# k-xlsx/huff-encoding

Measured on AMD Instinct MI355X. Metric: encode+decode GB/s on 1 GiB bytes at 1/2/4/8 MI355X; % HBM roofline, higher is better.
Workload: dtype u8; 1 GPU; 1 GiB uniform bytes (BASELINE configs[1]), encode+decode, bit-exact; bytes_per_gpu=1073741824, global_bytes=1073741824, compressed_bytes_per_gpu=1073741824, parallelism=shard1

## Files before the change

huff-encoding_amd/csrc/device/indexless.hip:

```cpp
#include <algorithm>

#include "segwalk.hpp"

namespace huff::dev {

namespace {

constexpr int kThreads = 256;

struct Seg {
    const uint8_t* comp;
    uint64_t comp_bytes;
    uint64_t B;
    uint64_t S;
    uint64_t nseg;
    const uint32_t* lut;
    uint32_t K;
    unsigned long long* wtot;
};

__device__ __forceinline__ void load_prim(uint32_t* plut, const Seg& g) {
    for (uint32_t i = threadIdx.x; i < (1u << g.K); i += blockDim.x) plut[i] = g.lut[i];
    __syncthreads();
}
// ... 180 lines not shown
template <class Step>
__device__ __forceinline__ void fix_list_body(const Seg& g, const PackedRecs& R, uint64_t* __restrict__ x,
                                              unsigned int* __restrict__ flags, const uint32_t* __restrict__ list,
                                              uint32_t* __restrict__ chain, const Step& step) {
    const uint64_t firsts = (g.nseg - 1) / kThreads;
    const uint64_t n = firsts + __builtin_nontemporal_load(flags + kFixRounds);
    for (uint64_t j = static_cast<uint64_t>(blockIdx.x) * blockDim.x + threadIdx.x; j < n;
         j += static_cast<uint64_t>(gridDim.x) * blockDim.x) {
        const uint64_t i = j < firsts ? (j + 1) * kThreads : list[j - firsts];
        fix_one(g, R, x, flags, 0, i, step, chain, flags + kFixRounds + 1);
    }
}
__global__ __launch_bounds__(kThreads) void k_fix_list(Seg g, PackedRecs R, uint64_t* __restrict__ x,
                                                       unsigned int* __restrict__ flags,
                                                       const uint32_t* __restrict__ list, uint32_t* __restrict__ chain,
                                                       FixTabs f) {
    extern __shared__ uint32_t plut[];
    if (f.wt) {
        fix_list_body(g, R, x, flags, list, chain, load_len_step(f, plut));
    } else {
        load_prim(plut, g);
        fix_list_body(g, R, x, flags, list, chain, LutStep{Lut{plut, g.lut, g.K}});
    }
}

constexpr int kChainThreads = 1024;
template <class Step>
__device__ __forceinline__ void fix_chain_body(const Seg& g, const PackedRecs& R, uint64_t* __restrict__ x,
                                               unsigned int* __restrict__ flags, uint32_t* __restrict__ chain,
                                               const Step& step);
__global__ __launch_bounds__(kChainThreads) void k_fix_chain(Seg g, PackedRecs R, uint64_t* __restrict__ x,
                                                             unsigned int* __restrict__ flags,
                                                             uint32_t* __restrict__ chain, FixTabs f) {
    if (__builtin_nontemporal_load(flags + kFixRounds + 1) == 0) return;
    extern __shared__ uint32_t plut[];
    if (f.wt) {
        fix_chain_body(g, R, x, flags, chain, load_len_step(f, plut));
    } else {
        load_prim(plut, g);
        fix_chain_body(g, R, x, flags, chain, LutStep{Lut{plut, g.lut, g.K}});
    }
}
template <class Step>
__device__ __forceinline__ void fix_chain_body(const Seg& g, const PackedRecs& R, uint64_t* __restrict__ x,
                                               unsigned int* __restrict__ flags, uint32_t* __restrict__ chain,
                                               const Step& step) {
    __shared__ uint32_t n_sh;
    uint32_t cur = 0;
    for (;;) {
        unsigned int* cnt = flags + kFixRounds + 1 + cur;
        unsigned int* ncnt = flags + kFixRounds + 2 - cur;
        if (threadIdx.x == 0) n_sh = atomicAdd(cnt, 0u);
        __syncthreads();
        const uint32_t n = n_sh;
        if (n == 0) break;
        const uint32_t* list = chain + static_cast<uint64_t>(cur) * g.nseg;
        uint32_t* nl = chain + static_cast<uint64_t>(cur ^ 1u) * g.nseg;
        for (uint32_t j = threadIdx.x; j < n; j += blockDim.x) fix_one(g, R, x, flags, 0, list[j], step, nl, ncnt);
        __syncthreads();
        if (threadIdx.x == 0) {
            atomicExch(cnt, 0u);
            atomicAdd(flags + kFixRounds + 3, n);
        }
        cur ^= 1u;
    }
}

__global__ void k_settle(Seg g, uint64_t* __restrict__ s, uint64_t* __restrict__ x, uint64_t* __restrict__ c,
                         uint32_t* __restrict__ tm, const unsigned int* __restrict__ flags) {
    if (__builtin_nontemporal_load(flags + kFixRounds - 1) == 0) return;
    extern __shared__ uint32_t plut[];
    load_prim(plut, g);
    if (threadIdx.x != 0) return;
    const BitSrc src{reinterpret_cast<const uint32_t*>(g.comp), g.comp, g.comp_bytes};
    const Lut lut{plut, g.lut, g.K};
    for (uint64_t i = 1; i < g.nseg; ++i) {
        const uint64_t ns = x[i - 1];
        if (ns == s[i]) continue;
        const uint64_t end = (i + 1 == g.nseg) ? g.B : ((i + 1) * g.S < g.B ? (i + 1) * g.S : g.B);
        BitReader rd;
        rd.seek(src, ns);
        uint64_t cnt = 0;
        while (rd.pos < end) {
            if (!step(rd, src, lut, g.B)) break;
            ++cnt;
        }
        s[i] = ns;
        x[i] = rd.pos;
        if (g.wtot) g.wtot[i / kThreads] += cnt - c[i];
        c[i] = cnt;
        tm[i] = kNoMerge;
    }
}

__global__ __launch_bounds__(kThreads) void k_emit(Seg g, const uint64_t* __restrict__ s,
                                                   const uint64_t* __restrict__ c, const uint64_t* __restrict__ off,
                                                   uint8_t* __restrict__ out) {
    extern __shared__ uint32_t plut[];
    load_prim(plut, g);
    const uint64_t i = static_cast<uint64_t>(blockIdx.x) * blockDim.x + threadIdx.x;
    if (i >= g.nseg) return;
    const uint64_t cnt = c[i];
    if (cnt == 0) return;
    const BitSrc src{reinterpret_cast<const uint32_t*>(g.comp), g.comp, g.comp_bytes};
    const Lut lut{plut, g.lut, g.K};
    BitReader rd;
    rd.seek(src, s[i]);
    uint8_t* o = out + off[i];
    for (uint64_t j = 0; j < cnt; ++j) {
        const uint32_t e = rd.peek(src, lut);
        rd.advance(src, (e >> 8) & 0xFFu);
        o[j] = static_cast<uint8_t>(e);
    }
}

Seg make_seg(const IndexlessArgs& a) {
    return Seg{a.comp, a.comp_bytes, a.valid_bits, a.seg_bits, a.nseg, a.lut, a.lut_bits, a.wtot};
}


constexpr uint32_t kSampStride = (kSampMax + 1) & ~1u;
constexpr uint32_t kSampNone = 0xFFFFu;
struct SampWords {
    uint32_t d[kSampStride / 2];
};
typedef uint32_t u32x4_a4 __attribute__((ext_vector_type(4), aligned(4)));
__device__ __forceinline__ SampWords samp_load(const uint16_t* samp, uint64_t i) {
    SampWords w;
    const uint32_t* p = reinterpret_cast<const uint32_t*>(samp + i * kSampStride);
    constexpr uint32_t kD = kSampStride / 2;
    uint32_t k = 0;
#pragma unroll
    for (; k + 4 <= kD; k += 4) {
        const u32x4_a4 v = *reinterpret_cast<const u32x4_a4*>(p + k);
        w.d[k] = v.x;
        w.d[k + 1] = v.y;
        w.d[k + 2] = v.z;
        w.d[k + 3] = v.w;
    }
#pragma unroll
    for (; k < kD; ++k) w.d[k] = p[k];
    return w;
}
__device__ __forceinline__ void samp_store(uint16_t* samp, uint64_t i, const SampWords& w) {
    uint32_t* p = reinterpret_cast<uint32_t*>(samp + i * kSampStride);
    constexpr uint32_t kD = kSampStride / 2;
    uint32_t k = 0;
#pragma unroll
    for (; k + 4 <= kD; k += 4)
        *reinterpret_cast<u32x4_a4*>(p + k) = u32x4_a4{w.d[k], w.d[k + 1], w.d[k + 2], w.d[k + 3]};
#pragma unroll
    for (; k < kD; ++k) p[k] = w.d[k];
}
__device__ __forceinline__ uint32_t samp_get(const SampWords& w, uint32_t k) {
    uint32_t d = 0;
#pragma unroll
    for (uint32_t j = 0; j < kSampStride / 2; ++j) d |= w.d[j] & (j == (k >> 1) ? ~0u : 0u);
    return (d >> (16 * (k & 1))) & 0xFFFFu;
}
__device__ __forceinline__ uint32_t samp_slot(const SampWords& w, uint32_t k) {
    return (w.d[k >> 1] >> (16 * (k & 1))) & 0xFFFFu;
}
__device__ __forceinline__ void samp_pick(const SampWords& w, uint32_t nsamp, uint32_t u, uint32_t& idx,
                                          uint32_t& rel) {
    idx = 0;
    rel = 0;
    uint32_t cum = 0;
#pragma unroll
    for (uint32_t k = 0; k < kSampMax; ++k) {
        const uint32_t v = samp_slot(w, k);
        const bool valid = k < nsamp && v != kSampNone;
        cum += valid ? v >> 8 : 0u;
        const bool ok = valid && cum <= u;
        idx = ok ? cum : idx;
        rel = ok ? kSampBits * (k + 1) + (v & 0xFFu) : rel;
    }
}


template <bool SLOW>
__global__ __launch_bounds__(kThreads) void k_spec_lds(IndexlessArgs a) {
    extern __shared__ __attribute__((aligned(16))) uint32_t lds[];
    WaveStamps ws;
    HUFF_STAMP(ws, 0);
    TabLoad tl;
    issue_tables(a, tl);
    const Staged st = with_l2(stage_block(a, lds + tables_words(a), a.lead_bits), a, lds);
    const uint16_t* stab = store_tables(a, tl, lds);
    const uint16_t* wtab = a.wtab ? stab : nullptr;
    __syncthreads();
    HUFF_STAMP(ws, 1);
    const uint64_t i0 = static_cast<uint64_t>(blockIdx.x) * blockDim.x + threadIdx.x;
    const bool live = i0 < a.nseg;
    const uint64_t i = live ? i0 : a.nseg - 1;
    const uint32_t K = a.stab_bits, Kg = a.lut_bits;
    const uint64_t B = a.valid_bits;
    const uint64_t start = i * a.seg_bits;
    const uint64_t end = (i + 1 == a.nseg) ? B : (start + a.seg_bits < B ? start + a.seg_bits : B);
    Cursor c;
    uint64_t cur = start, cnt = 0;
    if (a.lead_bits && start) {
        uint64_t p = start > a.lead_bits ? start - a.lead_bits : 0;
        c.init(st, p);
#ifndef HUFF_LEAD_MULTI
#define HUFF_LEAD_MULTI 1
#endif
#if HUFF_LEAD_MULTI
        if (wtab) {
            for (;;) {
                uint32_t U, N, q[kChunkSteps];
                c.multi_chunk<SLOW>(U, N, q, wtab, stab, K, a.lut, Kg);
                if (p + U < start) {
                    p += U;
                    continue;
                }
                uint32_t back = 0;
#pragma unroll
                for (int k = 0; k < kChunkSteps; ++k) {
                    const uint32_t u = q[k] & 0xFFFFu;
                    back = p + u < start ? u : back;
                }
                p += back;
                c.init(st, p);
                break;
            }
        }
#endif
        for (;;) {
            uint32_t L[kChunkSteps];
            c.chunk<SLOW>(L, stab, K, a.lut, Kg);
            uint64_t ex = ~0ull;
#pragma unroll
            for (int k = 0; k < kChunkSteps; ++k) {
                p += L[k];
                ex = (ex == ~0ull && p >= start) ? p : ex;
            }
            if (ex != ~0ull) {
                cur = ex < B ? ex : B;
                break;
            }
        }
    }
    c.init(st, cur);
    SampWords sw;
#pragma unroll
    for (uint32_t j = 0; j < kSampStride / 2; ++j) sw.d[j] = 0xFFFFFFFFu;
    uint32_t next_k = 1;
    uint64_t next_bit = (a.nsamp && live) ? start + kSampBits : ~0ull;
    uint64_t last_idx = 0;
    const uint64_t entry = cur;
    auto note_sample = [&]() {
        if (cur >= next_bit) {
            const uint64_t off = cur - next_bit, didx = cnt - last_idx;
            const bool ok = off < 256 && didx < 255;
            const uint32_t v16 = ok ? static_cast<uint32_t>(off | (didx << 8)) : kSampNone;
            const uint32_t k = next_k - 1, sh = 16 * (k & 1);
#pragma unroll
            for (uint32_t j = 0; j < kSampStride / 2; ++j) {
                const uint32_t m = j == (k >> 1) ? 0xFFFFu << sh : 0u;
                sw.d[j] = (sw.d[j] & ~m) | ((v16 << sh) & m);
            }
            last_idx = ok ? cnt : last_idx;
            next_bit = ++next_k <= a.nsamp ? next_bit + kSampBits : ~0ull;
        }
    };
    if (wtab) {
        const uint64_t span = static_cast<uint64_t>(kChunkSteps) * (a.max_len > K ? a.max_len : K);
        while (cur + span < end) {
            uint32_t U, N;
            c.multi_chunk<SLOW>(U, N, wtab, stab, K, a.lut, Kg);
            cur += U;
            cnt += N;
            note_sample();
        }
    }
    HUFF_STAMP(ws, 2);
    for (;;) {
        uint32_t L[kChunkSteps];
        c.chunk<SLOW>(L, stab, K, a.lut, Kg);
        uint64_t p = cur, ex = ~0ull;
        uint32_t ec = 0;
#pragma unroll
        for (int k = 0; k < kChunkSteps; ++k) {
            p += L[k];
            const bool hit = ex == ~0ull && p >= end;
            ex = hit ? p : ex;
            ec = hit ? static_cast<uint32_t>(k + 1) : ec;
        }
        if (ex != ~0ull) {
            cnt += ec;
            if (ex > B) {
                ex = B;
                --cnt;
            }
            cur = ex;
            break;
        }
        cur = p;
        cnt += kChunkSteps;
        note_sample();
    }
    HUFF_STAMP(ws, 3);
    if (live)
        samp_store(a.samp, i, sw);

    __shared__ uint32_t ex_w[kThreads / 64];
    const uint32_t cur_rel = static_cast<uint32_t>(cur - st.base);
    const uint32_t prev_rel = static_cast<uint32_t>(__shfl_up(static_cast<int>(cur_rel), 1));
    if ((threadIdx.x & 63) == 63) ex_w[threadIdx.x >> 6] = cur_rel;
    __syncthreads();
    const uint64_t cur0 = cur;
    uint64_t s_out = entry;
    uint32_t tm_out = 0;
    int32_t dl_out = 0;
    HUFF_STAMP(ws, 4);
    const uint64_t ns = !threadIdx.x ? entry
                        : st.base + ((threadIdx.x & 63) ? prev_rel : ex_w[(threadIdx.x >> 6) - 1]);
    if (ns != entry) {
        Cursor ca_;
        ca_.init(st, ns);
        uint64_t pa = ns, na = 0;
        uint64_t pk = 0;
        uint32_t ik = 0, cum = 0, k = 0;
        auto next_sample = [&]() {
            while (pa > pk) {
                const uint32_t v = k < a.nsamp ? samp_get(sw, k) : kSampNone;
                ++k;
                if (v != kSampNone) {
                    cum += v >> 8;
                    pk = start + kSampBits * k + (v & 0xFFu);
                    ik = cum;
                } else if (k >= a.nsamp) {
                    pk = ~0ull;
                }
            }
        };
        next_sample();
        for (;;) {
            uint32_t L[kChunkSteps];
            ca_.chunk<SLOW>(L, stab, K, a.lut, Kg);
            uint64_t p = pa;
            int hit = -1, ex = -1;
            uint64_t pex = 0;
#pragma unroll
            for (int j = 0; j < kChunkSteps; ++j) {
                p += L[j];
                hit = (hit < 0 && ex < 0 && p == pk) ? j : hit;
                const bool e = ex < 0 && hit < 0 && p >= end;
                ex = e ? j : ex;
                pex = e ? p : pex;
            }
            if (hit >= 0) {
                const uint64_t t = na + static_cast<uint64_t>(hit) + 1;
                tm_out = static_cast<uint32_t>(t);
                dl_out = static_cast<int32_t>(static_cast<int64_t>(t) - static_cast<int64_t>(ik));
                cnt = static_cast<uint64_t>(static_cast<int64_t>(cnt) + dl_out);
                break;
            }
            if (ex >= 0) {
                cnt = na + static_cast<uint64_t>(ex) + 1;
                if (pex > B) {
                    pex = B;
                    --cnt;
                }
                cur = pex;
                tm_out = kNoMerge;
                break;
            }
            pa = p;
            na += kChunkSteps;
            next_sample();
        }
        s_out = ns;
        if (live && tm_out == kNoMerge && cur != cur0 && i + 1 < a.nseg &&
            ((i + 1) % kThreads) != 0 && a.fixlist)
            a.fixlist[atomicAdd(a.flags + kFixRounds, 1u)] = static_cast<uint32_t>(i + 1);
    }
    HUFF_STAMP(ws, 5);
    ws.flush(a.stamps, static_cast<uint64_t>(blockIdx.x) * (kThreads / 64) + (threadIdx.x >> 6));
    if (a.wtot) {
        __shared__ uint32_t wsum[kThreads / 64];
        const uint32_t incl = wave_scan_incl(live ? static_cast<uint32_t>(cnt) : 0u);
        if ((threadIdx.x & 63) == 63) wsum[threadIdx.x >> 6] = incl;
        __syncthreads();
        if (threadIdx.x == 0) {
            uint64_t tot = 0;
#pragma unroll
            for (int w = 0; w < kThreads / 64; ++w) tot += wsum[w];
            a.wtot[blockIdx.x] = tot;
        }
    }
    if (!live) return;
    a.rec[i] = rec_pack(SegRec{s_out, cnt, tm_out, dl_out}, i, a.seg_bits);
    if (threadIdx.x == kThreads - 1 || i + 1 == a.nseg || (tm_out == kNoMerge && cur != cur0)) a.x[i] = cur;
}

template <bool SLOW>
__device__ __forceinline__ uint64_t walk(const Staged& st, uint64_t pos, uint32_t n, const uint16_t* stab, uint32_t K,
                                         const uint32_t* glut, uint32_t Kg) {
    Cursor c;
    c.init(st, pos);
    while (n) {
        uint32_t L[kChunkSteps];
        c.chunk<SLOW>(L, stab, K, glut, Kg);
#pragma unroll
        for (int k = 0; k < kChunkSteps; ++k) pos += static_cast<uint32_t>(k) < n ? L[k] : 0u;
        n = n > kChunkSteps ? n - kChunkSteps : 0u;
    }
    return pos;
}

template <bool SLOW>
__global__ __launch_bounds__(kThreads) void k_mark_lds(IndexlessArgs a, const uint64_t* __restrict__ off,
                                                       uint64_t* __restrict__ sub_abs, uint32_t shift) {
    extern __shared__ __attribute__((aligned(16))) uint32_t lds[];
    TabLoad tl;
    issue_tables(a, tl);
    const Staged st = with_l2(stage_block(a, lds + tables_words(a)), a, lds);
    const uint16_t* stab = store_tables(a, tl, lds);
    __syncthreads();
    const uint64_t i = static_cast<uint64_t>(blockIdx.x) * blockDim.x + threadIdx.x;
    if (i >= a.nseg) return;
    const uint32_t K = a.stab_bits, Kg = a.lut_bits;
    const uint64_t j0 = off[i];
    const SegRec v = rec_unpack(a.rec[i], i, a.seg_bits);
    const uint64_t cnt = v.c;
    const uint64_t step = 1ull << shift;
    uint64_t m = (j0 + step - 1) & ~(step - 1);
    if (m >= j0 + cnt) return;
    const uint64_t s_true = v.s;
    const uint64_t s_spec = i * a.seg_bits;
    const uint32_t tm = v.tm;
    const int64_t dl = v.dl;
    const SampWords sw = samp_load(a.samp, i);
    for (; m < j0 + cnt; m += step) {
        const uint64_t t = m - j0;
        uint64_t pos;
        if (tm == kNoMerge || t < tm) {
            pos = walk<SLOW>(st, s_true, static_cast<uint32_t>(t), stab, K, a.lut, Kg);
        } else {
            const uint32_t u = static_cast<uint32_t>(static_cast<int64_t>(t) - dl);
            uint32_t idx, rel;
            samp_pick(sw, a.nsamp, u, idx, rel);
            pos = rel ? walk<SLOW>(st, s_spec + rel, u - idx, stab, K, a.lut, Kg)
                      : walk<SLOW>(st, s_true, static_cast<uint32_t>(t), stab, K, a.lut, Kg);
        }
        sub_abs[m >> shift] = pos;
    }
}

__global__ __launch_bounds__(kThreads) void k_mark_lite(IndexlessArgs a, const uint64_t* __restrict__ off,
                                                        const unsigned long long* __restrict__ woff,
                                                        uint64_t* __restrict__ sub_abs, uint64_t sub_cap,
                                                        uint32_t* __restrict__ mark32,
                                                        uint32_t* __restrict__ task_seg) {
    const uint64_t i = static_cast<uint64_t>(blockIdx.x) * blockDim.x + threadIdx.x;
    const SegRec v = rec_unpack(i < a.nseg ? a.rec[i] : 0, i, a.seg_bits);
    uint64_t j0, cnt = i < a.nseg ? v.c : 0;
    if (woff) {
        __shared__ uint32_t wsum[kThreads / 64];
        const uint32_t incl = wave_scan_incl(static_cast<uint32_t>(cnt));
        if ((threadIdx.x & 63) == 63) wsum[threadIdx.x >> 6] = incl;
        __syncthreads();
        uint32_t pre = 0;
#pragma unroll
        for (uint32_t w = 0; w < kThreads / 64; ++w) pre += w < (threadIdx.x >> 6) ? wsum[w] : 0u;
        j0 = woff[blockIdx.x] + pre + incl - static_cast<uint32_t>(cnt);
        if (i >= a.nseg) return;
    } else {
        if (i >= a.nseg) return;
        j0 = off[i];
    }
    uint64_t m = (j0 + kIdx - 1) & ~static_cast<uint64_t>(kIdx - 1);
    const uint64_t m_end = j0 + cnt < sub_cap * kIdx ? j0 + cnt : sub_cap * kIdx;
    if (m >= m_end) return;
    const uint64_t s_true = v.s;
    const uint64_t s_spec = i * a.seg_bits;
    const uint32_t tm = v.tm;
    const int64_t dl = v.dl;
    const SampWords sw = samp_load(a.samp, i);
    for (; m < m_end; m += kIdx) {
        const uint32_t t = static_cast<uint32_t>(m - j0);
        uint64_t pos;
        uint32_t skip;
        if (tm == kNoMerge || t < tm) {
            pos = s_true;
            skip = t;
        } else {
            const uint32_t u = static_cast<uint32_t>(static_cast<int64_t>(t) - dl);
            uint32_t idx, rel;
            samp_pick(sw, a.nsamp, u, idx, rel);
            pos = rel ? s_spec + rel : s_true;
            skip = rel ? u - idx : t;
        }
        if (mark32) {
            mark32[m / kIdx] = skip | (static_cast<uint32_t>(pos - s_spec) << 10) |
                               (static_cast<uint32_t>(i & 0x7FFu) << 21);
            if ((m % kTaskSym) == 0) task_seg[m / kTaskSym] = static_cast<uint32_t>(i);
        } else {
            sub_abs[m / kIdx] = pos | (static_cast<uint64_t>(skip) << 48);
        }
    }
}

__global__ __launch_bounds__(kThreads) void k_rec_counts(const uint64_t* __restrict__ rec, uint64_t* __restrict__ c,
                                                         uint64_t n) {
    const uint64_t i = static_cast<uint64_t>(blockIdx.x) * blockDim.x + threadIdx.x;
    if (i < n) c[i] = rec[i] & 0xFFFFu;
}

}

hipError_t launch_indexless_mark_lite(const IndexlessArgs& a, const uint64_t* off, const unsigned long long* woff,
                                      uint64_t* sub_abs, uint64_t sub_cap, hipStream_t st, uint32_t* mark32,
                                      uint32_t* task_seg) {
    if (a.nseg == 0) return hipSuccess;
    if (!a.samp || !a.rec || (!off && !woff) || (!mark32 != !task_seg)) return hipErrorInvalidValue;
    launch_k(k_mark_lite, dim3((a.nseg + kThreads - 1) / kThreads), dim3(kThreads), 0, st, a, off, woff,
                       sub_abs, sub_cap < (~0ull / kIdx) ? sub_cap : (~0ull / kIdx), mark32, task_seg);
    return hipGetLastError();
}

static size_t lds_staged_bytes(const IndexlessArgs& a, uint32_t segs) {
    return static_cast<size_t>((((((1u << a.stab_bits) + 1) / 2) + 3) & ~3u) + a.l2_words) * 4 +
           ((segs * a.seg_bits + 7) / 8 + (a.lead_bits + 7) / 8 + 128 + 15) / 16 * 16;
}

static bool use_staged(const IndexlessArgs& a) {
    return a.stab && a.stab_bits && a.max_len <= 32 && a.seg_bits < 1024 &&
           lds_staged_bytes(a, kThreads) <= 160 * 1024;
}

hipError_t launch_indexless_mark(const IndexlessArgs& a, const uint64_t* off, uint64_t* sub_abs, uint32_t shift,
                                 hipStream_t st) {
    if (a.nseg == 0) return hipSuccess;
    if (!use_staged(a) || !a.samp || !a.rec) return hipErrorInvalidValue;
    const bool slow = a.max_len > a.stab_bits;
    IndexlessArgs m = a;
    m.wtab = nullptr;
    launch_k(slow ? k_mark_lds<true> : k_mark_lds<false>, dim3((m.nseg + kThreads - 1) / kThreads),
                       dim3(kThreads), lds_staged_bytes(m, kThreads), st, m, off, sub_abs, shift);
    return hipGetLastError();
}

bool indexless_staged(const IndexlessArgs& a) { return use_staged(a); }

hipError_t launch_indexless_spec(const IndexlessArgs& a, hipStream_t st) {
// ... 59 lines not shown
```

huff-encoding_amd/csrc/device/segwalk.hpp:

```cpp
#pragma once

#include "bitreader.hpp"

namespace huff::dev {

struct Staged {
    const uint32_t* w;
    uint64_t base;
    const uint32_t* l2;
    uint32_t l2e = 0;
    bool nofill = false;
    bool dense = false;
};

template <int N>
__device__ __forceinline__ void keep_loads(uint4 (&v)[N]) {
#pragma unroll
    for (int k = 0; k < N; ++k) asm volatile("" : "+v"(v[k].x), "+v"(v[k].y), "+v"(v[k].z), "+v"(v[k].w));
}

template <uint32_t NSEG = 256, class A>
__device__ __forceinline__ Staged stage_block(const A& a, uint32_t* w, uint32_t lead = 0) {
    constexpr uint32_t kT = 256;
    const uint64_t seg0 = static_cast<uint64_t>(blockIdx.x) * NSEG;
    const uint64_t bit_lo = seg0 * a.seg_bits - (seg0 * a.seg_bits < lead ? seg0 * a.seg_bits : lead);
    const uint64_t seg_end = seg0 + NSEG < a.nseg ? seg0 + NSEG : a.nseg;
    const uint64_t bit_hi = seg_end * a.seg_bits < a.valid_bits ? seg_end * a.seg_bits : a.valid_bits;
    const uint64_t byte_lo = (bit_lo >> 3) & ~15ull;
    uint64_t byte_hi = ((bit_hi + 7) >> 3) + 64;
    if (byte_hi > a.comp_bytes) byte_hi = a.comp_bytes;
    const uint32_t nbytes = static_cast<uint32_t>(byte_hi - byte_lo);
    const uint32_t np = (nbytes + 8 + 15) / 16;
    const auto rs = buf_rsrc(a.comp + byte_lo, (nbytes + 15) & ~15u);
    uint4* w4 = reinterpret_cast<uint4*>(w);
    for (uint32_t p0 = threadIdx.x; p0 < np; p0 += 8 * kT) {
        uint4 v[8];
#pragma unroll
        for (int k = 0; k < 8; ++k) v[k] = buf_ld16(rs, (p0 + k * kT) * 16);
        keep_loads(v);
#pragma unroll
        for (int k = 0; k < 8; ++k)
            if (p0 + k * kT < np) w4[p0 + k * kT] = v[k];
    }
    return Staged{w, byte_lo * 8, nullptr};
}

constexpr int kChunkSteps = 8;
#ifndef HUFF_WALK_R
#define HUFF_WALK_R 1
#endif
constexpr bool kWalkR = HUFF_WALK_R != 0;

struct Cursor {
    const uint32_t* w;
    const uint32_t* l2;
    uint64_t buf;
    uint32_t X, rp, nextw;
    uint32_t l2e;
    bool nofill, dense;
    __device__ __forceinline__ void init(const Staged& st, uint64_t p) {
        w = st.w;
        l2 = st.l2;
        l2e = st.l2e;
        nofill = st.nofill;
        dense = st.dense;
        const uint64_t rel = p - st.base;
        rp = static_cast<uint32_t>(rel >> 5);
        const uint32_t sh = static_cast<uint32_t>(rel & 31);
        buf = static_cast<uint64_t>(__builtin_bswap32(w[rp]) << sh) << 32;
        X = 32 - sh;
        rp += 1;
        nextw = __builtin_bswap32(w[rp]);
    }
    __device__ __forceinline__ void refill() {
        buf |= (static_cast<uint64_t>(nextw) << 32) >> (X & 63);
        rp += (X & 32) ? 0u : 1u;
        X |= 32;
        nextw = __builtin_bswap32(w[rp]);
    }
    template <bool SLOW>
    __device__ __forceinline__ uint32_t step(const uint16_t* stab, uint32_t K, const uint32_t* glut, uint32_t Kg) {
        return step_entry<SLOW>(stab[static_cast<uint32_t>(buf >> 32) >> (32 - K)], K, glut, Kg);
    }
    __device__ __forceinline__ uint32_t dense_len(uint32_t e, uint32_t K) const {
        const uint32_t s = (e & 0x7Fu) | ((e >> 8) << 7);
        const uint32_t j = (static_cast<uint32_t>(buf >> 32) << K) >> (32 - l2e);
        return reinterpret_cast<const uint8_t*>(l2)[(e & kSsSlow) ? (s << l2e) + j : 0u];
    }
    template <bool SLOW>
    __device__ __forceinline__ uint32_t step_entry(uint32_t e, uint32_t K, const uint32_t* glut, uint32_t Kg) {
        if (SLOW && dense) {
            const uint32_t l1 = dense_len(e, K);
            const uint32_t len = (e & kSsSlow) ? l1 : (e & 63u);
            buf <<= len;
            X -= len;
            return len;
        }
        if (SLOW && (e & kSsSlow) && l2 && l2e) {
            if (!nofill) refill();
            const uint32_t s = (e & 0x7Fu) | ((e >> 8) << 7);
            const uint32_t j = (static_cast<uint32_t>(buf >> 32) << K) >> (32 - l2e);
            const uint32_t l1 = reinterpret_cast<const uint8_t*>(l2)[(s << l2e) + j];
            buf <<= l1;
            X -= l1;
            if (!nofill) refill();
            return l1;
        }
        if (SLOW && (e & kSsSlow) && l2) {
            refill();
            const uint32_t d = l2[(e & 0x7Fu) | ((e >> 8) << 7)];
            const uint32_t E = d & 31u;
            const uint32_t j = (static_cast<uint32_t>(buf >> 32) << K) >> (32 - E);
            const uint32_t l1 = reinterpret_cast<const uint8_t*>(l2)[(d >> 5) + j];
            buf <<= l1;
            X -= l1;
            refill();
            return l1;
        }
        if (SLOW && (e & kSsSlow)) {
            refill();
            uint32_t e1 = glut[static_cast<uint32_t>(buf >> (64 - Kg))];
            uint32_t d = Kg;
            while (e1 & kLutPtr) {
                const uint32_t idx = static_cast<uint32_t>((buf >> (56 - d)) & 0xFFu);
                e1 = glut[(e1 & ~kLutPtr) + idx];
                d += 8;
            }
            const uint32_t l1 = (e1 >> 8) & 0xFFu;
            buf <<= l1;
            X -= l1;
            refill();
            return l1;
        }
        buf <<= (e & 63u);
        X -= e;
        return e & 63u;
    }
    __device__ __forceinline__ static uint32_t refill_steps(uint32_t K) {
        return !kWalkR || K > 10 ? 0x55u : K > 8 ? 0x49u : 0x11u;
    }
    template <bool SLOW>
    __device__ __forceinline__ void chunk(uint32_t (&L)[kChunkSteps], const uint16_t* stab, uint32_t K,
                                          const uint32_t* glut, uint32_t Kg) {
        const uint32_t rs = SLOW ? 0x55u : refill_steps(K);
#pragma unroll
        for (int k = 0; k < kChunkSteps; ++k) {
            if ((rs >> k) & 1u) refill();
            L[k] = step<SLOW>(stab, K, glut, Kg);
        }
    }
    template <bool SLOW>
    __device__ __forceinline__ void multi_chunk(uint32_t& U, uint32_t& N, const uint16_t* wtab, const uint16_t* stab,
                                                uint32_t K, const uint32_t* glut, uint32_t Kg) {
        U = 0;
        N = 0;
        const uint32_t rs = SLOW ? 0x55u : refill_steps(K);
#pragma unroll
        for (int k = 0; k < kChunkSteps; ++k) {
            if ((rs >> k) & 1u) refill();
            const uint32_t e = wtab[static_cast<uint32_t>(buf >> 32) >> (32 - K)];
            if (SLOW && dense) {
                const uint32_t l1 = dense_len(e, K);
                const bool slow = (e & kSsSlow) != 0;
                const uint32_t u = slow ? l1 : (e >> 8) & 15u;
                buf <<= u;
                X -= u;
                U += u;
                N += slow ? 1u : e >> 12;
            } else if (SLOW && (e & kSsSlow)) {
                U += step_entry<SLOW>(e, K, glut, Kg);
                N += 1;
            } else {
                const uint32_t u = (e >> 8) & 15u;
                buf <<= u;
                X -= u;
                U += u;
                N += e >> 12;
            }
        }
    }
    template <bool SLOW>
    __device__ __forceinline__ void multi_chunk(uint32_t& U, uint32_t& N, uint32_t (&q)[kChunkSteps],
                                                const uint16_t* wtab, const uint16_t* stab, uint32_t K,
                                                const uint32_t* glut, uint32_t Kg) {
        uint32_t Q = 0;
        const uint32_t rs = SLOW ? 0x55u : refill_steps(K);
#pragma unroll
        for (int k = 0; k < kChunkSteps; ++k) {
            if ((rs >> k) & 1u) refill();
            const uint32_t e = wtab[static_cast<uint32_t>(buf >> 32) >> (32 - K)];
            if (SLOW && (e & kSsSlow)) {
                Q += step_entry<SLOW>(e, K, glut, Kg) + (1u << 16);
            } else {
                const uint32_t u = (e >> 8) & 15u;
                buf <<= u;
                X -= u;
                Q += u + ((e >> 12) << 16);
            }
            q[k] = Q;
        }
        U = Q & 0xFFFFu;
        N = Q >> 16;
    }
};

template <class A>
__device__ __forceinline__ uint32_t stab_words(const A& a) {
    return ((((1u << a.stab_bits) + 1) / 2) + 3) & ~3u;
}
template <class A>
__device__ __forceinline__ uint32_t tables_words(const A& a) {
    return stab_words(a) + a.l2_words;
}
constexpr uint32_t kTabPieces = 2, kL2Pieces = 6;
constexpr uint32_t kL2MaxWords = 4 * 256 * kL2Pieces;
struct TabLoad {
    uint4 t[kTabPieces];
    uint4 l[kL2Pieces];
};
template <class A>
__device__ __forceinline__ void issue_tables(const A& a, TabLoad& tl) {
    const uint32_t words = ((1u << a.stab_bits) + 1) / 2;
    const auto r1 = buf_rsrc(a.wtab ? a.wtab : a.stab, words * 4);
#pragma unroll
    for (uint32_t k = 0; k < kTabPieces; ++k) tl.t[k] = buf_ld16(r1, (threadIdx.x + 256 * k) * 16);
    if (a.l2_words) {
        const auto r2 = buf_rsrc(a.l2, a.l2_words * 4);
#pragma unroll
        for (uint32_t k = 0; k < kL2Pieces; ++k) tl.l[k] = buf_ld16(r2, (threadIdx.x + 256 * k) * 16);
    }
}
template <class A>
__device__ __forceinline__ const uint16_t* store_tables(const A& a, const TabLoad& tl, uint32_t* lds) {
    const uint32_t sp = stab_words(a) / 4, lp = (a.l2_words + 3) / 4;
    uint4* l4 = reinterpret_cast<uint4*>(lds);
#pragma unroll
    for (uint32_t k = 0; k < kTabPieces; ++k)
        if (threadIdx.x + 256 * k < sp) l4[threadIdx.x + 256 * k] = tl.t[k];
    if (a.l2_words) {
#pragma unroll
        for (uint32_t k = 0; k < kL2Pieces; ++k)
            if (threadIdx.x + 256 * k < lp) l4[sp + threadIdx.x + 256 * k] = tl.l[k];
    }
    return reinterpret_cast<const uint16_t*>(lds);
}
template <class A>
__device__ __forceinline__ const uint16_t* load_stab(const A& a, uint32_t* lds) {
    TabLoad tl;
    issue_tables(a, tl);
    return store_tables(a, tl, lds);
}
template <class A>
__device__ __forceinline__ Staged with_l2(Staged st, const A& a, const uint32_t* lds) {
    st.l2 = a.l2_words ? lds + stab_words(a) : nullptr;
    st.l2e = a.l2_words ? a.l2_e : 0u;
    st.nofill = st.l2e && a.max_len <= 16;
    st.dense = st.nofill && a.l2_dense;
    return st;
}

}
```

Measured before the change: 1239 GB/s.

## Walk segments with 32-bit block-relative positions and an alignbit window cursor

Replaces the 64-bit bit-buffer cursor in the speculative segment walk with a WalkCursor that keeps two 32-bit words and builds the decode window with alignbit. All positions, counts and sample bookkeeping become 32-bit offsets relative to the staged base. Sample recording changes from masked per-slot insertion to a shift-in push, and the multi-symbol step packs length and count into one running total. The aim is fewer 64-bit ALU ops and VGPRs on the hot decode loop, at the cost of new position arithmetic that must stay exact, including the clamp of the valid-bit limit to 31 bits.

After: 1237 GB/s. No clear change (-0.1%).

```diff
diff --git a/huff-encoding_amd/csrc/device/indexless.hip b/huff-encoding_amd/csrc/device/indexless.hip
--- a/huff-encoding_amd/csrc/device/indexless.hip
+++ b/huff-encoding_amd/csrc/device/indexless.hip
@@ -356,6 +356,12 @@
 #pragma unroll
     for (; k < kD; ++k) p[k] = w.d[k];
 }
+__device__ __forceinline__ void samp_push(SampWords& w, uint32_t v16) {
+    constexpr uint32_t kD = kSampStride / 2;
+#pragma unroll
+    for (uint32_t j = 0; j + 1 < kD; ++j) w.d[j] = __builtin_amdgcn_alignbit(w.d[j + 1], w.d[j], 16);
+    w.d[kD - 1] = __builtin_amdgcn_alignbit(v16, w.d[kD - 1], 16);
+}
 __device__ __forceinline__ uint32_t samp_get(const SampWords& w, uint32_t k) {
     uint32_t d = 0;
 #pragma unroll
@@ -398,13 +404,16 @@
     const bool live = i0 < a.nseg;
     const uint64_t i = live ? i0 : a.nseg - 1;
     const uint32_t K = a.stab_bits, Kg = a.lut_bits;
-    const uint64_t B = a.valid_bits;
-    const uint64_t start = i * a.seg_bits;
-    const uint64_t end = (i + 1 == a.nseg) ? B : (start + a.seg_bits < B ? start + a.seg_bits : B);
-    Cursor c;
-    uint64_t cur = start, cnt = 0;
-    if (a.lead_bits && start) {
-        uint64_t p = start > a.lead_bits ? start - a.lead_bits : 0;
+    const uint64_t start64 = i * a.seg_bits;
+    const uint32_t start = static_cast<uint32_t>(start64 - st.base);
+    const uint64_t B64 = a.valid_bits - st.base;
+    const uint32_t B = B64 < 0x7FFFFFFFull ? static_cast<uint32_t>(B64) : 0x7FFFFFFFu;
+    const uint32_t seg_end = start + static_cast<uint32_t>(a.seg_bits);
+    const uint32_t end = (i + 1 == a.nseg) ? B : (seg_end < B ? seg_end : B);
+    WalkCursor c;
+    uint32_t cur = start, cnt = 0;
+    if (a.lead_bits && start64) {
+        uint32_t p = start64 > a.lead_bits ? start - a.lead_bits : 0u;
         c.init(st, p);
 #ifndef HUFF_LEAD_MULTI
 #define HUFF_LEAD_MULTI 1
@@ -412,19 +421,14 @@
 #if HUFF_LEAD_MULTI
         if (wtab) {
             for (;;) {
-                uint32_t U, N, q[kChunkSteps];
-                c.multi_chunk<SLOW>(U, N, q, wtab, stab, K, a.lut, Kg);
-                if (p + U < start) {
-                    p += U;
+                uint32_t q[kChunkSteps];
+                c.multi_chunk<SLOW>(q, wtab, K, a.lut, Kg);
+                if (q[kChunkSteps - 1] < start) {
+                    p = q[kChunkSteps - 1];
                     continue;
                 }
-                uint32_t back = 0;
-#pragma unroll
-                for (int k = 0; k < kChunkSteps; ++k) {
-                    const uint32_t u = q[k] & 0xFFFFu;
-                    back = p + u < start ? u : back;
-                }
-                p += back;
+#pragma unroll
+                for (int k = 0; k < kChunkSteps; ++k) p = q[k] < start ? q[k] : p;
                 c.init(st, p);
                 break;
             }
@@ -433,13 +437,13 @@
         for (;;) {
             uint32_t L[kChunkSteps];
             c.chunk<SLOW>(L, stab, K, a.lut, Kg);
-            uint64_t ex = ~0ull;
+            uint32_t ex = ~0u;
 #pragma unroll
             for (int k = 0; k < kChunkSteps; ++k) {
                 p += L[k];
-                ex = (ex == ~0ull && p >= start) ? p : ex;
-            }
-            if (ex != ~0ull) {
+                ex = (ex == ~0u && p >= start) ? p : ex;
+            }
+            if (ex != ~0u) {
                 cur = ex < B ? ex : B;
                 break;
             }
@@ -450,31 +454,25 @@
 #pragma unroll
     for (uint32_t j = 0; j < kSampStride / 2; ++j) sw.d[j] = 0xFFFFFFFFu;
     uint32_t next_k = 1;
-    uint64_t next_bit = (a.nsamp && live) ? start + kSampBits : ~0ull;
-    uint64_t last_idx = 0;
-    const uint64_t entry = cur;
+    uint32_t next_bit = (a.nsamp && live) ? start + kSampBits : ~0u;
+    uint32_t last_idx = 0;
+    const uint32_t entry = cur;
     auto note_sample = [&]() {
         if (cur >= next_bit) {
-            const uint64_t off = cur - next_bit, didx = cnt - last_idx;
+            const uint32_t off = cur - next_bit, didx = cnt - last_idx;
             const bool ok = off < 256 && didx < 255;
-            const uint32_t v16 = ok ? static_cast<uint32_t>(off | (didx << 8)) : kSampNone;
-            const uint32_t k = next_k - 1, sh = 16 * (k & 1);
-#pragma unroll
-            for (uint32_t j = 0; j < kSampStride / 2; ++j) {
-                const uint32_t m = j == (k >> 1) ? 0xFFFFu << sh : 0u;
-                sw.d[j] = (sw.d[j] & ~m) | ((v16 << sh) & m);
-            }
+            samp_push(sw, ok ? off | (didx << 8) : kSampNone);
             last_idx = ok ? cnt : last_idx;
-            next_bit = ++next_k <= a.nsamp ? next_bit + kSampBits : ~0ull;
+            next_bit = ++next_k <= a.nsamp ? next_bit + kSampBits : ~0u;
         }
     };
     if (wtab) {
-        const uint64_t span = static_cast<uint64_t>(kChunkSteps) * (a.max_len > K ? a.max_len : K);
+        const uint32_t span = kChunkSteps * (a.max_len > K ? a.max_len : K);
         while (cur + span < end) {
-            uint32_t U, N;
-            c.multi_chunk<SLOW>(U, N, wtab, stab, K, a.lut, Kg);
-            cur += U;
-            cnt += N;
+            const uint32_t T = c.multi_chunk<SLOW>(wtab, K, a.lut, Kg);
+            const uint32_t p = c.pos();
+            cnt += (T - (p - cur)) >> 4;
+            cur = p;
             note_sample();
         }
     }
@@ -482,16 +480,16 @@
     for (;;) {
         uint32_t L[kChunkSteps];
         c.chunk<SLOW>(L, stab, K, a.lut, Kg);
-        uint64_t p = cur, ex = ~0ull;
+        uint32_t p = cur, ex = ~0u;
         uint32_t ec = 0;
 #pragma unroll
         for (int k = 0; k < kChunkSteps; ++k) {
             p += L[k];
-            const bool hit = ex == ~0ull && p >= end;
+            const bool hit = ex == ~0u && p >= end;
             ex = hit ? p : ex;
             ec = hit ? static_cast<uint32_t>(k + 1) : ec;
         }
-        if (ex != ~0ull) {
+        if (ex != ~0u) {
             cnt += ec;
             if (ex > B) {
                 ex = B;
@@ -505,26 +503,25 @@
         note_sample();
     }
     HUFF_STAMP(ws, 3);
+    for (uint32_t k = next_k - 1; k < kSampStride; ++k) samp_push(sw, kSampNone);
     if (live)
         samp_store(a.samp, i, sw);
 
     __shared__ uint32_t ex_w[kThreads / 64];
-    const uint32_t cur_rel = static_cast<uint32_t>(cur - st.base);
-    const uint32_t prev_rel = static_cast<uint32_t>(__shfl_up(static_cast<int>(cur_rel), 1));
-    if ((threadIdx.x & 63) == 63) ex_w[threadIdx.x >> 6] = cur_rel;
+    const uint32_t prev = static_cast<uint32_t>(__shfl_up(static_cast<int>(cur), 1));
+    if ((threadIdx.x & 63) == 63) ex_w[threadIdx.x >> 6] = cur;
     __syncthreads();
-    const uint64_t cur0 = cur;
-    uint64_t s_out = entry;
+    const uint32_t cur0 = cur;
+    uint32_t s_out = entry;
     uint32_t tm_out = 0;
     int32_t dl_out = 0;
     HUFF_STAMP(ws, 4);
-    const uint64_t ns = !threadIdx.x ? entry
-                        : st.base + ((threadIdx.x & 63) ? prev_rel : ex_w[(threadIdx.x >> 6) - 1]);
+    const uint32_t ns = !threadIdx.x ? entry : (threadIdx.x & 63) ? prev : ex_w[(threadIdx.x >> 6) - 1];
     if (ns != entry) {
-        Cursor ca_;
+        WalkCursor ca_;
         ca_.init(st, ns);
-        uint64_t pa = ns, na = 0;
-        uint64_t pk = 0;
+        uint32_t pa = ns, na = 0;
+        uint32_t pk = 0;
         uint32_t ik = 0, cum = 0, k = 0;
         auto next_sample = [&]() {
             while (pa > pk) {
@@ -535,7 +532,7 @@
                     pk = start + kSampBits * k + (v & 0xFFu);
                     ik = cum;
                 } else if (k >= a.nsamp) {
-                    pk = ~0ull;
+                    pk = ~0u;
                 }
             }
         };
@@ -543,9 +540,9 @@
         for (;;) {
             uint32_t L[kChunkSteps];
             ca_.chunk<SLOW>(L, stab, K, a.lut, Kg);
-            uint64_t p = pa;
+            uint32_t p = pa;
             int hit = -1, ex = -1;
-            uint64_t pex = 0;
+            uint32_t pex = 0;
 #pragma unroll
             for (int j = 0; j < kChunkSteps; ++j) {
                 p += L[j];
@@ -555,14 +552,13 @@
                 pex = e ? p : pex;
             }
             if (hit >= 0) {
-                const uint64_t t = na + static_cast<uint64_t>(hit) + 1;
-                tm_out = static_cast<uint32_t>(t);
-                dl_out = static_cast<int32_t>(static_cast<int64_t>(t) - static_cast<int64_t>(ik));
-                cnt = static_cast<uint64_t>(static_cast<int64_t>(cnt) + dl_out);
+                tm_out = na + static_cast<uint32_t>(hit) + 1;
+                dl_out = static_cast<int32_t>(tm_out - ik);
+                cnt += static_cast<uint32_t>(dl_out);
                 break;
             }
             if (ex >= 0) {
-                cnt = na + static_cast<uint64_t>(ex) + 1;
+                cnt = na + static_cast<uint32_t>(ex) + 1;
                 if (pex > B) {
                     pex = B;
                     --cnt;
@@ -584,7 +580,7 @@
     ws.flush(a.stamps, static_cast<uint64_t>(blockIdx.x) * (kThreads / 64) + (threadIdx.x >> 6));
     if (a.wtot) {
         __shared__ uint32_t wsum[kThreads / 64];
-        const uint32_t incl = wave_scan_incl(live ? static_cast<uint32_t>(cnt) : 0u);
+        const uint32_t incl = wave_scan_incl(live ? cnt : 0u);
         if ((threadIdx.x & 63) == 63) wsum[threadIdx.x >> 6] = incl;
         __syncthreads();
         if (threadIdx.x == 0) {
@@ -595,8 +591,8 @@
         }
     }
     if (!live) return;
-    a.rec[i] = rec_pack(SegRec{s_out, cnt, tm_out, dl_out}, i, a.seg_bits);
-    if (threadIdx.x == kThreads - 1 || i + 1 == a.nseg || (tm_out == kNoMerge && cur != cur0)) a.x[i] = cur;
+    a.rec[i] = rec_pack(SegRec{st.base + s_out, cnt, tm_out, dl_out}, i, a.seg_bits);
+    if (threadIdx.x == kThreads - 1 || i + 1 == a.nseg || (tm_out == kNoMerge && cur != cur0)) a.x[i] = st.base + cur;
 }
 
 template <bool SLOW>
diff --git a/huff-encoding_amd/csrc/device/segwalk.hpp b/huff-encoding_amd/csrc/device/segwalk.hpp
--- a/huff-encoding_amd/csrc/device/segwalk.hpp
+++ b/huff-encoding_amd/csrc/device/segwalk.hpp
@@ -1,17 +1,10 @@
 #pragma once
 
 #include "bitreader.hpp"
+#include "walk_cursor.hpp"
 
 namespace huff::dev {
 
-struct Staged {
-    const uint32_t* w;
-    uint64_t base;
-    const uint32_t* l2;
-    uint32_t l2e = 0;
-    bool nofill = false;
-    bool dense = false;
-};
 
 template <int N>
 __device__ __forceinline__ void keep_loads(uint4 (&v)[N]) {
@@ -44,165 +37,6 @@
     }
     return Staged{w, byte_lo * 8, nullptr};
 }
-
-constexpr int kChunkSteps = 8;
-#ifndef HUFF_WALK_R
-#define HUFF_WALK_R 1
-#endif
-constexpr bool kWalkR = HUFF_WALK_R != 0;
-
-struct Cursor {
-    const uint32_t* w;
-    const uint32_t* l2;
-    uint64_t buf;
-    uint32_t X, rp, nextw;
-    uint32_t l2e;
-    bool nofill, dense;
-    __device__ __forceinline__ void init(const Staged& st, uint64_t p) {
-        w = st.w;
-        l2 = st.l2;
-        l2e = st.l2e;
-        nofill = st.nofill;
-        dense = st.dense;
-        const uint64_t rel = p - st.base;
-        rp = static_cast<uint32_t>(rel >> 5);
-        const uint32_t sh = static_cast<uint32_t>(rel & 31);
-        buf = static_cast<uint64_t>(__builtin_bswap32(w[rp]) << sh) << 32;
-        X = 32 - sh;
-        rp += 1;
-        nextw = __builtin_bswap32(w[rp]);
-    }
-    __device__ __forceinline__ void refill() {
-        buf |= (static_cast<uint64_t>(nextw) << 32) >> (X & 63);
-        rp += (X & 32) ? 0u : 1u;
-        X |= 32;
-        nextw = __builtin_bswap32(w[rp]);
-    }
-    template <bool SLOW>
-    __device__ __forceinline__ uint32_t step(const uint16_t* stab, uint32_t K, const uint32_t* glut, uint32_t Kg) {
-        return step_entry<SLOW>(stab[static_cast<uint32_t>(buf >> 32) >> (32 - K)], K, glut, Kg);
-    }
-    __device__ __forceinline__ uint32_t dense_len(uint32_t e, uint32_t K) const {
-        const uint32_t s = (e & 0x7Fu) | ((e >> 8) << 7);
-        const uint32_t j = (static_cast<uint32_t>(buf >> 32) << K) >> (32 - l2e);
-        return reinterpret_cast<const uint8_t*>(l2)[(e & kSsSlow) ? (s << l2e) + j : 0u];
-    }
-    template <bool SLOW>
-    __device__ __forceinline__ uint32_t step_entry(uint32_t e, uint32_t K, const uint32_t* glut, uint32_t Kg) {
-        if (SLOW && dense) {
-            const uint32_t l1 = dense_len(e, K);
-            const uint32_t len = (e & kSsSlow) ? l1 : (e & 63u);
-            buf <<= len;
-            X -= len;
-            return len;
-        }
-        if (SLOW && (e & kSsSlow) && l2 && l2e) {
-            if (!nofill) refill();
-            const uint32_t s = (e & 0x7Fu) | ((e >> 8) << 7);
-            const uint32_t j = (static_cast<uint32_t>(buf >> 32) << K) >> (32 - l2e);
-            const uint32_t l1 = reinterpret_cast<const uint8_t*>(l2)[(s << l2e) + j];
-            buf <<= l1;
-            X -= l1;
-            if (!nofill) refill();
-            return l1;
-        }
-        if (SLOW && (e & kSsSlow) && l2) {
-            refill();
-            const uint32_t d = l2[(e & 0x7Fu) | ((e >> 8) << 7)];
-            const uint32_t E = d & 31u;
-            const uint32_t j = (static_cast<uint32_t>(buf >> 32) << K) >> (32 - E);
-            const uint32_t l1 = reinterpret_cast<const uint8_t*>(l2)[(d >> 5) + j];
-            buf <<= l1;
-            X -= l1;
-            refill();
-            return l1;
-        }
-        if (SLOW && (e & kSsSlow)) {
-            refill();
-            uint32_t e1 = glut[static_cast<uint32_t>(buf >> (64 - Kg))];
-            uint32_t d = Kg;
-            while (e1 & kLutPtr) {
-                const uint32_t idx = static_cast<uint32_t>((buf >> (56 - d)) & 0xFFu);
-                e1 = glut[(e1 & ~kLutPtr) + idx];
-                d += 8;
-            }
-            const uint32_t l1 = (e1 >> 8) & 0xFFu;
-            buf <<= l1;
-            X -= l1;
-            refill();
-            return l1;
-        }
-        buf <<= (e & 63u);
-        X -= e;
-        return e & 63u;
-    }
-    __device__ __forceinline__ static uint32_t refill_steps(uint32_t K) {
-        return !kWalkR || K > 10 ? 0x55u : K > 8 ? 0x49u : 0x11u;
-    }
-    template <bool SLOW>
-    __device__ __forceinline__ void chunk(uint32_t (&L)[kChunkSteps], const uint16_t* stab, uint32_t K,
-                                          const uint32_t* glut, uint32_t Kg) {
-        const uint32_t rs = SLOW ? 0x55u : refill_steps(K);
-#pragma unroll
-        for (int k = 0; k < kChunkSteps; ++k) {
-            if ((rs >> k) & 1u) refill();
-            L[k] = step<SLOW>(stab, K, glut, Kg);
-        }
-    }
-    template <bool SLOW>
-    __device__ __forceinline__ void multi_chunk(uint32_t& U, uint32_t& N, const uint16_t* wtab, const uint16_t* stab,
-                                                uint32_t K, const uint32_t* glut, uint32_t Kg) {
-        U = 0;
-        N = 0;
-        const uint32_t rs = SLOW ? 0x55u : refill_steps(K);
-#pragma unroll
-        for (int k = 0; k < kChunkSteps; ++k) {
-            if ((rs >> k) & 1u) refill();
-            const uint32_t e = wtab[static_cast<uint32_t>(buf >> 32) >> (32 - K)];
-            if (SLOW && dense) {
-                const uint32_t l1 = dense_len(e, K);
-                const bool slow = (e & kSsSlow) != 0;
-                const uint32_t u = slow ? l1 : (e >> 8) & 15u;
-                buf <<= u;
-                X -= u;
-                U += u;
-                N += slow ? 1u : e >> 12;
-            } else if (SLOW && (e & kSsSlow)) {
-                U += step_entry<SLOW>(e, K, glut, Kg);
-                N += 1;
-            } else {
-                const uint32_t u = (e >> 8) & 15u;
-                buf <<= u;
-                X -= u;
-                U += u;
-                N += e >> 12;
-            }
-        }
-    }
-    template <bool SLOW>
-    __device__ __forceinline__ void multi_chunk(uint32_t& U, uint32_t& N, uint32_t (&q)[kChunkSteps],
-                                                const uint16_t* wtab, const uint16_t* stab, uint32_t K,
-                                                const uint32_t* glut, uint32_t Kg) {
-        uint32_t Q = 0;
-        const uint32_t rs = SLOW ? 0x55u : refill_steps(K);
-#pragma unroll
-        for (int k = 0; k < kChunkSteps; ++k) {
-            if ((rs >> k) & 1u) refill();
-            const uint32_t e = wtab[static_cast<uint32_t>(buf >> 32) >> (32 - K)];
-            if (SLOW && (e & kSsSlow)) {
-                Q += step_entry<SLOW>(e, K, glut, Kg) + (1u << 16);
-            } else {
-                const uint32_t u = (e >> 8) & 15u;
-                buf <<= u;
-                X -= u;
-                Q += u + ((e >> 12) << 16);
-            }
-            q[k] = Q;
-        }
-        U = Q & 0xFFFFu;
-        N = Q >> 16;
-    }
-};
 
 template <class A>
 __device__ __forceinline__ uint32_t stab_words(const A& a) {
diff --git a/huff-encoding_amd/csrc/device/walk_cursor.hpp b/huff-encoding_amd/csrc/device/walk_cursor.hpp
--- /dev/null
+++ b/huff-encoding_amd/csrc/device/walk_cursor.hpp
@@ -0,0 +1,313 @@
+#pragma once
+
+#include "kernels.hpp"
+
+#ifndef __HIPCC__
+static inline uint32_t __builtin_amdgcn_alignbit(uint32_t hi, uint32_t lo, uint32_t s) {
+    return static_cast<uint32_t>(((static_cast<uint64_t>(hi) << 32) | lo) >> (s & 31u));
+}
+#endif
+
+namespace huff::dev {
+
+struct Staged {
+    const uint32_t* w;
+    uint64_t base;
+    const uint32_t* l2;
+    uint32_t l2e = 0;
+    bool nofill = false;
+    bool dense = false;
+};
+
+constexpr int kChunkSteps = 8;
+#ifndef HUFF_WALK_R
+#define HUFF_WALK_R 1
+#endif
+constexpr bool kWalkR = HUFF_WALK_R != 0;
+
+struct Cursor {
+    const uint32_t* w;
+    const uint32_t* l2;
+    uint64_t buf;
+    uint32_t X, rp, nextw;
+    uint32_t l2e;
+    bool nofill, dense;
+    __device__ __forceinline__ void init(const Staged& st, uint64_t p) {
+        w = st.w;
+        l2 = st.l2;
+        l2e = st.l2e;
+        nofill = st.nofill;
+        dense = st.dense;
+        const uint64_t rel = p - st.base;
+        rp = static_cast<uint32_t>(rel >> 5);
+        const uint32_t sh = static_cast<uint32_t>(rel & 31);
+        buf = static_cast<uint64_t>(__builtin_bswap32(w[rp]) << sh) << 32;
+        X = 32 - sh;
+        rp += 1;
+        nextw = __builtin_bswap32(w[rp]);
+    }
+    __device__ __forceinline__ void refill() {
+        buf |= (static_cast<uint64_t>(nextw) << 32) >> (X & 63);
+        rp += (X & 32) ? 0u : 1u;
+        X |= 32;
+        nextw = __builtin_bswap32(w[rp]);
+    }
+    template <bool SLOW>
+    __device__ __forceinline__ uint32_t step(const uint16_t* stab, uint32_t K, const uint32_t* glut, uint32_t Kg) {
+        return step_entry<SLOW>(stab[static_cast<uint32_t>(buf >> 32) >> (32 - K)], K, glut, Kg);
+    }
+    __device__ __forceinline__ uint32_t dense_len(uint32_t e, uint32_t K) const {
+        const uint32_t s = (e & 0x7Fu) | ((e >> 8) << 7);
+        const uint32_t j = (static_cast<uint32_t>(buf >> 32) << K) >> (32 - l2e);
+        return reinterpret_cast<const uint8_t*>(l2)[(e & kSsSlow) ? (s << l2e) + j : 0u];
+    }
+    template <bool SLOW>
+    __device__ __forceinline__ uint32_t step_entry(uint32_t e, uint32_t K, const uint32_t* glut, uint32_t Kg) {
+        if (SLOW && dense) {
+            const uint32_t l1 = dense_len(e, K);
+            const uint32_t len = (e & kSsSlow) ? l1 : (e & 63u);
+            buf <<= len;
+            X -= len;
+            return len;
+        }
+        if (SLOW && (e & kSsSlow) && l2 && l2e) {
+            if (!nofill) refill();
+            const uint32_t s = (e & 0x7Fu) | ((e >> 8) << 7);
+            const uint32_t j = (static_cast<uint32_t>(buf >> 32) << K) >> (32 - l2e);
+            const uint32_t l1 = reinterpret_cast<const uint8_t*>(l2)[(s << l2e) + j];
+            buf <<= l1;
+            X -= l1;
+            if (!nofill) refill();
+            return l1;
+        }
+        if (SLOW && (e & kSsSlow) && l2) {
+            refill();
+            const uint32_t d = l2[(e & 0x7Fu) | ((e >> 8) << 7)];
+            const uint32_t E = d & 31u;
+            const uint32_t j = (static_cast<uint32_t>(buf >> 32) << K) >> (32 - E);
+            const uint32_t l1 = reinterpret_cast<const uint8_t*>(l2)[(d >> 5) + j];
+            buf <<= l1;
+            X -= l1;
+            refill();
+            return l1;
+        }
+        if (SLOW && (e & kSsSlow)) {
+            refill();
+            uint32_t e1 = glut[static_cast<uint32_t>(buf >> (64 - Kg))];
+            uint32_t d = Kg;
+            while (e1 & kLutPtr) {
+                const uint32_t idx = static_cast<uint32_t>((buf >> (56 - d)) & 0xFFu);
+                e1 = glut[(e1 & ~kLutPtr) + idx];
+                d += 8;
+            }
+            const uint32_t l1 = (e1 >> 8) & 0xFFu;
+            buf <<= l1;
+            X -= l1;
+            refill();
+            return l1;
+        }
+        buf <<= (e & 63u);
+        X -= e;
+        return e & 63u;
+    }
+    __device__ __forceinline__ static uint32_t refill_steps(uint32_t K) {
+        return !kWalkR || K > 10 ? 0x55u : K > 8 ? 0x49u : 0x11u;
+    }
+    template <bool SLOW>
+    __device__ __forceinline__ void chunk(uint32_t (&L)[kChunkSteps], const uint16_t* stab, uint32_t K,
+                                          const uint32_t* glut, uint32_t Kg) {
+        const uint32_t rs = SLOW ? 0x55u : refill_steps(K);
+#pragma unroll
+        for (int k = 0; k < kChunkSteps; ++k) {
+            if ((rs >> k) & 1u) refill();
+            L[k] = step<SLOW>(stab, K, glut, Kg);
+        }
+    }
+    template <bool SLOW>
+    __device__ __forceinline__ void multi_chunk(uint32_t& U, uint32_t& N, const uint16_t* wtab, const uint16_t* stab,
+                                                uint32_t K, const uint32_t* glut, uint32_t Kg) {
+        U = 0;
+        N = 0;
+        const uint32_t rs = SLOW ? 0x55u : refill_steps(K);
+#pragma unroll
+        for (int k = 0; k < kChunkSteps; ++k) {
+            if ((rs >> k) & 1u) refill();
+            const uint32_t e = wtab[static_cast<uint32_t>(buf >> 32) >> (32 - K)];
+            if (SLOW && dense) {
+                const uint32_t l1 = dense_len(e, K);
+                const bool slow = (e & kSsSlow) != 0;
+                const uint32_t u = slow ? l1 : (e >> 8) & 15u;
+                buf <<= u;
+                X -= u;
+                U += u;
+                N += slow ? 1u : e >> 12;
+            } else if (SLOW && (e & kSsSlow)) {
+                U += step_entry<SLOW>(e, K, glut, Kg);
+                N += 1;
+            } else {
+                const uint32_t u = (e >> 8) & 15u;
+                buf <<= u;
+                X -= u;
+                U += u;
+                N += e >> 12;
+            }
+        }
+    }
+    template <bool SLOW>
+    __device__ __forceinline__ void multi_chunk(uint32_t& U, uint32_t& N, uint32_t (&q)[kChunkSteps],
+                                                const uint16_t* wtab, const uint16_t* stab, uint32_t K,
+                                                const uint32_t* glut, uint32_t Kg) {
+        uint32_t Q = 0;
+        const uint32_t rs = SLOW ? 0x55u : refill_steps(K);
+#pragma unroll
+        for (int k = 0; k < kChunkSteps; ++k) {
+            if ((rs >> k) & 1u) refill();
+            const uint32_t e = wtab[static_cast<uint32_t>(buf >> 32) >> (32 - K)];
+            if (SLOW && (e & kSsSlow)) {
+                Q += step_entry<SLOW>(e, K, glut, Kg) + (1u << 16);
+            } else {
+                const uint32_t u = (e >> 8) & 15u;
+                buf <<= u;
+                X -= u;
+                Q += u + ((e >> 12) << 16);
+            }
+            q[k] = Q;
+        }
+        U = Q & 0xFFFFu;
+        N = Q >> 16;
+    }
+};
+
+struct WalkCursor {
+    const uint32_t* w;
+    const uint32_t* l2;
+    uint32_t hi, lo, nextw, win;
+    uint32_t s, rp;
+    uint32_t l2e;
+    bool nofill, dense;
+    __device__ __forceinline__ void init(const Staged& st, uint32_t rel) {
+        w = st.w;
+        l2 = st.l2;
+        l2e = st.l2e;
+        nofill = st.nofill;
+        dense = st.dense;
+        const uint32_t m = (rel + 31) >> 5;
+        s = (0u - rel) & 31u;
+        hi = __builtin_bswap32(w[m ? m - 1 : 0]);
+        lo = __builtin_bswap32(w[m]);
+        rp = m + 1;
+        nextw = __builtin_bswap32(w[rp]);
+        win = __builtin_amdgcn_alignbit(hi, lo, s);
+    }
+    __device__ __forceinline__ uint32_t pos() const { return ((rp - 1) << 5) - s; }
+    __device__ __forceinline__ void refill() {
+        const bool adv = static_cast<int32_t>(s) < 0;
+        hi = adv ? lo : hi;
+        lo = adv ? nextw : lo;
+        rp += adv ? 1u : 0u;
+        s &= 31u;
+        win = __builtin_amdgcn_alignbit(hi, lo, s);
+        nextw = __builtin_bswap32(w[rp]);
+    }
+    __device__ __forceinline__ void take(uint32_t n) {
+        win <<= n;
+        s -= n;
+    }
+    __device__ __forceinline__ uint32_t dense_len(uint32_t e, uint32_t K) const {
+        const uint32_t t = (e & 0x7Fu) | ((e >> 8) << 7);
+        const uint32_t j = (win << K) >> (32 - l2e);
+        return reinterpret_cast<const uint8_t*>(l2)[(e & kSsSlow) ? (t << l2e) + j : 0u];
+    }
+    __device__ __forceinline__ uint32_t slow_step(uint32_t e, uint32_t K, const uint32_t* glut, uint32_t Kg) {
+        uint32_t l1;
+        if (l2 && l2e) {
+            if (!nofill) refill();
+            const uint32_t t = (e & 0x7Fu) | ((e >> 8) << 7);
+            const uint32_t j = (win << K) >> (32 - l2e);
+            l1 = reinterpret_cast<const uint8_t*>(l2)[(t << l2e) + j];
+            if (nofill) {
+                take(l1);
+                return l1;
+            }
+        } else if (l2) {
+            refill();
+            const uint32_t d = l2[(e & 0x7Fu) | ((e >> 8) << 7)];
+            const uint32_t E = d & 31u;
+            const uint32_t j = (win << K) >> (32 - E);
+            l1 = reinterpret_cast<const uint8_t*>(l2)[(d >> 5) + j];
+        } else {
+            refill();
+            uint32_t e1 = glut[win >> (32 - Kg)];
+            uint32_t d = Kg;
+            while (e1 & kLutPtr) {
+                const uint32_t idx = (d <= 24 ? win >> (24 - d) : win << (d - 24)) & 0xFFu;
+                e1 = glut[(e1 & ~kLutPtr) + idx];
+                d += 8;
+            }
+            l1 = (e1 >> 8) & 0xFFu;
+        }
+        s -= l1;
+        refill();
+        return l1;
+    }
+    template <bool SLOW>
+    __device__ __forceinline__ uint32_t step_entry(uint32_t e, uint32_t K, const uint32_t* glut, uint32_t Kg) {
+        if (SLOW && dense) {
+            const uint32_t l1 = dense_len(e, K);
+            const uint32_t len = (e & kSsSlow) ? l1 : (e & 63u);
+            take(len);
+            return len;
+        }
+        if (SLOW && (e & kSsSlow)) return slow_step(e, K, glut, Kg);
+        take(e & 63u);
+        return e & 63u;
+    }
+    template <bool SLOW>
+    __device__ __forceinline__ void chunk(uint32_t (&L)[kChunkSteps], const uint16_t* stab, uint32_t K,
+                                          const uint32_t* glut, uint32_t Kg) {
+        const uint32_t rs = SLOW ? 0x55u : Cursor::refill_steps(K);
+#pragma unroll
+        for (int k = 0; k < kChunkSteps; ++k) {
+            if ((rs >> k) & 1u) refill();
+            L[k] = step_entry<SLOW>(stab[win >> (32 - K)], K, glut, Kg);
+        }
+    }
+    template <bool SLOW>
+    __device__ __forceinline__ uint32_t window(const uint16_t* wtab, uint32_t K, const uint32_t* glut, uint32_t Kg) {
+        const uint32_t e = wtab[win >> (32 - K)];
+        if (SLOW && dense) {
+            const uint32_t l1 = dense_len(e, K);
+            const bool slow = (e & kSsSlow) != 0;
+            take(slow ? l1 : (e >> 8) & 15u);
+            return slow ? l1 + 16u : e >> 8;
+        }
+        if (SLOW && (e & kSsSlow)) return slow_step(e, K, glut, Kg) + 16u;
+        take((e >> 8) & 15u);
+        return e >> 8;
+    }
+    template <bool SLOW>
+    __device__ __forceinline__ uint32_t multi_chunk(const uint16_t* wtab, uint32_t K, const uint32_t* glut,
+                                                    uint32_t Kg) {
+        uint32_t T = 0;
+        const uint32_t rs = SLOW ? 0x55u : Cursor::refill_steps(K);
+#pragma unroll
+        for (int k = 0; k < kChunkSteps; ++k) {
+            if ((rs >> k) & 1u) refill();
+            T += window<SLOW>(wtab, K, glut, Kg);
+        }
+        return T;
+    }
+    template <bool SLOW>
+    __device__ __forceinline__ void multi_chunk(uint32_t (&q)[kChunkSteps], const uint16_t* wtab, uint32_t K,
+                                                const uint32_t* glut, uint32_t Kg) {
+        const uint32_t rs = SLOW ? 0x55u : Cursor::refill_steps(K);
+#pragma unroll
+        for (int k = 0; k < kChunkSteps; ++k) {
+            if ((rs >> k) & 1u) refill();
+            window<SLOW>(wtab, K, glut, Kg);
+            q[k] = pos();
+        }
+    }
+};
+
+}
```
